# lauradarcy/gym-craftingworld

Measured on AMD Instinct MI355X. Metric: env-steps/sec at 65536 envs, 1/2/4/8 MI355X; bit-exact vs CPU ref, higher is better.
Workload: dtype u8

## Files before the change

gym_craftingworld_amd/_lib.py:

```python
import ctypes as C
import os

_HERE = os.path.dirname(os.path.abspath(__file__))
LIB_PATH = os.path.join(_HERE, 'libcraftingworld.so')


def lib_path():
    return os.environ.get('CW_LIB_PATH') or LIB_PATH

CW_ABI_VERSION = 5
CW_MT_N = 624
CW_MAX_TASKS = 16
CW_MAX_MENUS = 256

CW_OK, CW_ERR_INVALID, CW_ERR_HIP, CW_ERR_STATE = 0, -1, -2, -3
CW_OBS_STATE, CW_OBS_PIXELS_FULL, CW_OBS_PIXELS_DIRTY = 0, 1, 2
CW_ACT_I32, CW_ACT_I64, CW_ACT_U8 = 0, 1, 2
CW_RASTER_RAY, CW_RASTER_ALT = 0, 1


class cw_task_menu(C.Structure):
    _fields_ = [('n_selected', C.c_int32), ('number_of_tasks', C.c_int32), ('stacking', C.c_int32),
                ('reward_subset', C.c_int32), ('selected_bits', C.c_int32 * CW_MAX_TASKS)]

# ... 46 lines not shown
    'cw_imagine_masked': (C.c_int, [_VP, _VP, _VP, C.c_int32, _VP, _VP, _VP]),
    'cw_sample_state_masked': (C.c_int, [_VP, _VP, C.c_int32, _VP, _VP]),
    'cw_step': (C.c_int, [_VP, _VP, C.c_int, _VP]),
    'cw_step_many': (C.c_int, [_VP, _VP, C.c_int, C.c_int32, _VP]),
    'cw_rollout': (C.c_int, [_VP, _VP, C.c_int32, _VP, _VP, _VP]),
    'cw_render': (C.c_int, [_VP, _VP, _VP]),
    'cw_render_onehot': (C.c_int, [_VP, _VP, C.c_int32, _VP, _VP]),
    'cw_export_grid': (C.c_int, [_VP, _VP, _VP]),
    'cw_export_onehot': (C.c_int, [_VP, _VP, _VP]),
    'cw_export_onehot_of': (C.c_int, [_VP, C.c_int, _VP, _VP]),
    'cw_get_state': (C.c_int, [_VP, C.POINTER(cw_state_view)]),
    'cw_set_state': (C.c_int, [_VP, C.POINTER(cw_state_view)]),
    'cw_checkpoint_bytes': (C.c_size_t, [_VP]),
    'cw_checkpoint_save': (C.c_int, [_VP, _VP, C.c_size_t]),
    'cw_checkpoint_load': (C.c_int, [_VP, _VP, C.c_size_t]),
    'cw_profile_begin': (C.c_int, [_VP, C.c_int]),
    'cw_profile_end': (C.c_int, [_VP, C.POINTER(cw_profile)]),
    'cw_tuner': (C.c_int, [_VP, C.POINTER(cw_tuner_state)]),
    'cw_step_resident': (C.c_int, [_VP, C.c_int32, C.c_int32]),
    'cw_resident_stop': (C.c_int, [_VP]),
    'cw_render_kernel_name': (C.c_char_p, [_VP]),
    'cw_buffers': (C.c_int, [_VP, C.POINTER(cw_buffer_table)]),
    'cw_synchronize': (C.c_int, [_VP, _VP]),
    'cw_num_envs': (C.c_int, [_VP]),
    'cw_abi_version': (C.c_int, []),
    'cw_last_error': (C.c_char_p, []),
}
class cwh_guard(C.Structure):
    _fields_ = [('rate', C.c_double), ('rate_top', C.c_double), ('ms_sum', C.c_double), ('prev_mean', C.c_double), ('ref_ms', C.c_double),
                ('ref_prev', C.c_double), ('ms_n', C.c_int32), ('late', C.c_int32), ('good', C.c_int32), ('slowdowns', C.c_int32),
                ('probes', C.c_int32), ('probe_need', C.c_int32), ('recover_need', C.c_int32), ('probing', C.c_int32), ('recovering', C.c_int32)]


class cwh_tuning(C.Structure):
    _fields_ = [(f, C.c_int32) for f in ('render_chunk_rounds', 'step_envs_per_wave', 'gather', 'gather_max_size', 'small_frame_bytes',
                                         'small_blocks_per_cu', 'small_launch_mb', 'reset_blocks_per_cu', 'guard', 'verbose', 'lookahead',
                                         'la_period', 'rollout_segment', 'pad')] + \
              [(f, C.c_double) for f in ('head_notch', 'busy_notch', 'period_ns', 'rate_tbs')]


cwh_lookup = C.CFUNCTYPE(_VP, _VP, C.c_char_p)

CWH_GUARD_NONE, CWH_GUARD_SLOWDOWN, CWH_GUARD_TRIAL_UP, CWH_GUARD_TRIAL_KEPT, CWH_GUARD_TRIAL_UNDONE = range(5)
CWH_CKPT_SECTIONS = 22

HOST_HELPERS = {
    'cwh_mt_from_numpy': (C.c_int, [_VP, C.c_int]),
    'cwh_mt_to_numpy': (None, [_VP, C.c_int, _VP]),
    'cwh_mt_init_genrand': (None, [_VP, C.c_uint32]),
    'cwh_mt_untwist': (None, [_VP]),
    'cwh_mt_rewind': (None, [_VP, C.POINTER(C.c_int32), C.c_uint32]),
    'cwh_dlpack_make': (_VP, [_VP, C.c_int, C.c_int, C.c_int, C.c_int, C.POINTER(C.c_int64)]),
    'cwh_slots_to_grid': (None, [_VP, C.c_uint32, C.c_int, _VP]),
    'cwh_ckpt_section_bytes': (C.c_int, [C.c_int64, C.c_int32, C.c_int32, C.POINTER(C.c_size_t), C.POINTER(C.c_uint64)]),
    'cwh_guard_init': (None, [C.POINTER(cwh_guard), C.c_double]),
    'cwh_guard_step': (C.c_int, [C.POINTER(cwh_guard), C.c_double, C.c_double]),
    'cwh_sweep_periods': (None, [C.c_double, C.c_int32, C.c_double, C.c_double, C.POINTER(C.c_int32), C.POINTER(C.c_int32), C.POINTER(C.c_int32)]),
    'cwh_guard_scheduled_ms': (C.c_double, [C.c_double, C.c_int32, C.c_int32, C.c_double]),
    'cwh_la_adapt': (C.c_int32, [C.c_int32, C.c_int32, C.c_uint64, C.POINTER(C.c_int32)]),
    'cwh_read_tuning': (None, [cwh_lookup, _VP, C.POINTER(cwh_tuning)]),
}


def bind_host_helpers(lib):
    for name, (res, args) in HOST_HELPERS.items():
        fn = getattr(lib, name)
        fn.restype = res
        fn.argtypes = args
    return lib

_libs = {}
_lib = None


class CraftingWorldError(RuntimeError):
    pass


def load():
    global _lib
    path = lib_path()
    if path in _libs:
        _lib = _libs[path]
        return _lib
    if not os.path.exists(path):
        raise CraftingWorldError(
            'HIP extension %s is missing; build it (python -c "import __graft_entry__ as g; g.build()"). '
            'There is no CPU fallback.' % path)
    try:
        import torch
    except ImportError:
# ... 21 lines not shown
```

gym_craftingworld_amd/csrc/cw_engine.cpp:

```cpp
#include <hip/hip_runtime.h>

#include <cstdarg>
#include <climits>
#include <cstdio>
#include <cstdlib>
#include <cstring>
#include <new>
#include <algorithm>
#include <vector>

#include "../../include/craftingworld.h"
#include "cw_layout.h"
#include "cw_host.h"

extern "C" {
hipError_t cwk_launch_step(const CwParams *P, const CwTuning *T, const void *actions, int act_dtype, int obs_mode, int auto_reset, hipStream_t st,
                           hipEvent_t *ev);
hipError_t cwk_launch_refill(const CwParams *P, const CwTuning *T, int all_envs, hipStream_t st);
hipError_t cwk_launch_reset_all(const CwParams *P, const CwTuning *T, int obs_mode, hipStream_t st);
hipError_t cwk_launch_reset_masked(const CwParams *P, const CwTuning *T, const uint8_t *mask, int obs_mode, hipStream_t st);
hipError_t cwk_launch_imagine_masked(const CwParams *P, const CwTuning *T, const uint8_t *mask, const uint16_t *desired, int commit, int obs_mode,
                                     uint8_t *out_frames, uint8_t *out_onehot, hipStream_t st);
hipError_t cwk_launch_sample_state_masked(const CwParams *P, const CwTuning *T, const uint8_t *mask, int pooled, uint16_t *out_cells, hipStream_t st);
hipError_t cwk_launch_pool(const CwParams *P, const CwTuning *T, hipStream_t st);
hipError_t cwk_launch_seed(const CwParams *P, const uint32_t *seeds_dev, hipStream_t st);
hipError_t cwk_launch_resident(const CwParams *P, CwResident *R, uint32_t seq0, int paint_dirty, unsigned long long idle_ticks,
                               unsigned long long life_ticks, hipStream_t st);
hipError_t cwk_launch_render_onehot(const CwParams *P, const uint8_t *onehot, int n_states, uint16_t *out, hipStream_t st);
hipError_t cwk_launch_render_restore(const CwParams *P, const CwTuning *T, hipStream_t st);
hipError_t cwk_launch_rollout(const CwParams *P, const uint8_t *actions, int T, int32_t *rewards, uint8_t *dones, hipStream_t st);
hipError_t cwk_launch_render_ext(const CwParams *P, const CwTuning *T, uint8_t *out, hipStream_t st);
hipError_t cwk_launch_sweep_calib(const CwParams *P, const CwTuning *T, hipStream_t st);
void cwk_sweep_shape(const CwParams *P, const CwTuning *T, int *n_chunks, int *waves, int *jobs_per_wave);
hipError_t cwk_launch_idle(hipStream_t st);
hipError_t cwk_launch_export(const CwParams *P, const CwTuning *T, uint8_t *out, int onehot, int which, hipStream_t st);
}

#include <time.h>

static thread_local char g_err[512] = "";

static int fail(int code, const char *fmt, ...)
{
    va_list ap;
    va_start(ap, fmt);
    vsnprintf(g_err, sizeof(g_err), fmt, ap);
    va_end(ap);
    return code;
}

// ... 125 lines not shown
{
    void *p = nullptr;
    size_t bytes = count * sizeof(T);
    if (bytes == 0) bytes = 16;
    HIP_TRY(hipMalloc(&p, bytes));
    HIP_TRY(hipMemset(p, 0, bytes));
    e->allocs.push_back(p);
    *out = (T *)p;
    return CW_OK;
}

template <typename T>
static int host_alloc(cw_engine *e, T **out, size_t count)
{
    void *p = nullptr, *d = nullptr;
    size_t bytes = count * sizeof(T);
    if (bytes == 0) bytes = 16;
    HIP_TRY(hipHostMalloc(&p, bytes, hipHostMallocCoherent));
    e->host_allocs.push_back(p);
    memset(p, 0, bytes);
    HIP_TRY(hipHostGetDevicePointer(&d, p, 0));
    if (d != p) return fail(CW_ERR_HIP, "cw_create: mapped host memory has a different device address (no unified addressing)");
    *out = (T *)p;
    return CW_OK;
}

static void prof_free(cw_engine *e)
{
    for (hipEvent_t ev : e->prof_ev) (void)hipEventDestroy(ev);
    e->prof_ev.clear();
    e->prof_cap = e->prof_n = 0;
}

static int timed_render_stats(cw_engine *e, double *median, double *p90, double *mean = nullptr)
{
    enum { LAUNCHES = 24, SKIP = 4 };
    hipEvent_t evs[2 * LAUNCHES] = {};
    bool ok = true;
    for (hipEvent_t &ev : evs) ok = ok && hipEventCreate(&ev) == hipSuccess;
    for (int rep = 0; rep < LAUNCHES && ok; rep++)
        ok = hipEventRecord(evs[2 * rep], e->aux) == hipSuccess && cwk_launch_sweep_calib(&e->P, &e->tune, e->aux) == hipSuccess &&
             hipEventRecord(evs[2 * rep + 1], e->aux) == hipSuccess && cwk_launch_idle(e->aux) == hipSuccess;
    ok = ok && hipStreamSynchronize(e->aux) == hipSuccess;
    float ms[LAUNCHES];
    for (int rep = 0; rep < LAUNCHES && ok; rep++) ok = hipEventElapsedTime(&ms[rep], evs[2 * rep], evs[2 * rep + 1]) == hipSuccess;
    for (hipEvent_t &ev : evs) if (ev) (void)hipEventDestroy(ev);
    if (!ok) return fail(CW_ERR_HIP, "cw_create: render calibration failed");
    std::sort(ms + SKIP, ms + LAUNCHES);
    const int n = LAUNCHES - SKIP;
    *median = ms[SKIP + n / 2];
    *p90 = ms[SKIP + (9 * n) / 10 - 1];
    if (mean) { double acc = 0; for (int i = SKIP; i < LAUNCHES; i++) acc += ms[i]; *mean = acc / n; }
    return CW_OK;
}

static double sweep_period_ns(const cw_engine *e, double tb_per_s) { return (double)e->sweep_waves * 4096.0 / (tb_per_s * 1e12) * 1e9; }
static void set_sweep_rate(cw_engine *e, double tb_per_s)
{
    cwh_sweep_periods(tb_per_s, e->sweep_waves, e->head_notch, e->busy_notch, &e->tune.period16, &e->tune.period16_head, &e->tune.period16_busy);
}

static int calibrate_sweep(cw_engine *e)
{
    CwTuning &tn = e->tune;
    int n_chunks = 1, jobs_per_wave = 1;
    cwk_sweep_shape(&e->P, &tn, &n_chunks, &e->sweep_waves, &jobs_per_wave);
    e->sweep_jobs = (double)n_chunks * jobs_per_wave;
    if (e->tune_period_ns >= 0) {
        const double ns = e->tune_period_ns;
        set_sweep_rate(e, ns > 0 ? (double)e->sweep_waves * 4096.0 / (ns * 1e-9) * 1e-12 : 0.0);
        if (ns > 0) tn.period16 = (int)(ns * 1.6 + 0.5);
        return CW_OK;
    }
    set_sweep_rate(e, 7.0);
    if (e->host_actions) { set_sweep_rate(e, 0); return CW_OK; }
    if (e->obs_mode != CW_OBS_PIXELS_FULL || (double)e->n * e->P.frame_bytes < (double)(64ll << 20)) return CW_OK;
    static const double rates[] = {7.7, 7.4, 7.2, 7.0, 6.8, 6.6, 0.0};
    char log[1024] = "";
    size_t len = 0;
    int rc = CW_OK;
    double best_p90 = 0, med = 0, p90 = 0, mean = 0;
    rc = timed_render_stats(e, &med, &p90);
    set_sweep_rate(e, 6.4);
    if (rc == CW_OK) rc = timed_render_stats(e, &med, &p90);
    e->sweep_beside_ms = med - e->sweep_jobs * sweep_period_ns(e, 6.4) * 1e-6;
    if (e->tune_rate_tbs >= 0) e->sweep_rate = e->tune_rate_tbs;
    for (size_t i = 0; i < sizeof(rates) / sizeof(rates[0]) && rc == CW_OK && e->tune_rate_tbs < 0; i++) {
        set_sweep_rate(e, rates[i]);
        rc = timed_render_stats(e, &med, &p90, &mean);
        if (len < sizeof(log) - 56) len += (size_t)snprintf(log + len, sizeof(log) - len, " %.1f TB/s (%.0f ns): %.4f/%.4f/%.4f |", rates[i], tn.period16 / 1.6, med, p90, mean);
        if (rc == CW_OK && (best_p90 == 0 || p90 < 0.995 * best_p90)) { best_p90 = p90; e->sweep_rate = rates[i]; }
    }
    set_sweep_rate(e, e->sweep_rate);
    cwh_guard_init(&e->guard, e->sweep_rate);
    e->guard_on = rc == CW_OK && e->sweep_rate > 0 && e->auto_reset && e->tune_guard;
    if (e->guard_on)
        for (auto &smp : e->guard_ring)
            for (hipEvent_t &ev : smp.ev)
                if (hipEventCreate(&ev) != hipSuccess) e->guard_on = false;
    if (e->verbose)
        fprintf(stderr, "[craftingworld] sweep clock, ms per sweep (median/90th percentile/mean of 20; 0.0 TB/s = unclocked):%s -> %s%.0f ns\n", log,
                tn.period16 ? "" : "unclocked, ", tn.period16 / 1.6);
    return rc;
}

enum { CW_GUARD_EVERY = 64 };
static hipEvent_t *sweep_guard_tick(cw_engine *e, hipStream_t st)
{
    if (++e->guard_step % CW_GUARD_EVERY) return nullptr;
    while (e->guard_tail != e->guard_head && hipEventQuery(e->guard_ring[e->guard_tail % cw_engine::GUARD_RING].ev[5]) == hipSuccess) {
        cw_engine::GuardSample &smp = e->guard_ring[e->guard_tail++ % cw_engine::GUARD_RING];
        float ms = 0.f;
        if (hipEventElapsedTime(&ms, smp.ev[4], smp.ev[5]) != hipSuccess || ms <= 0.f || smp.period16 != e->tune.period16) continue;
        const double scheduled = cwh_guard_scheduled_ms(e->sweep_jobs, e->tune.period16, e->tune.period16_busy, e->sweep_beside_ms);
        const double rate_before = e->guard.rate, prev_mean = e->guard.prev_mean;
        const int recovering = e->guard.recovering;
        const int action = cwh_guard_step(&e->guard, ms, scheduled);
        if (e->guard.rate != rate_before) set_sweep_rate(e, e->guard.rate);
        if (e->verbose && action != CWH_GUARD_NONE) {
            static const char *what[] = {"", "three samples in a row late: a notch down", "trying a notch up", "the trial pays: kept", "the trial does not pay: undone"};
            fprintf(stderr, "[craftingworld] sweep clock: %s%s -- %.4f ms against %.4f scheduled (mean at the rate left %.4f): %.1f -> %.1f TB/s (%.0f ns)\n", what[action],
                    recovering ? " (on the way back to the best rate known)" : "", ms, scheduled, prev_mean, rate_before, e->guard.rate, e->tune.period16 / 1.6);
        }
    }
    if (e->guard_head - e->guard_tail >= (unsigned)cw_engine::GUARD_RING) return nullptr;
    cw_engine::GuardSample &slot = e->guard_ring[e->guard_head++ % cw_engine::GUARD_RING];
    slot.period16 = e->tune.period16;
    return slot.ev;
}

static void read_tuning(cw_engine *e)
{
    CwTuning &tn = e->tune;
    cwh_tuning t{};
    t.render_chunk_rounds = tn.render_chunk_rounds;
// ... 394 lines not shown
    if (!e->has_reset) return fail(CW_ERR_STATE, "cw_sample_state_masked called before cw_reset");
    DeviceGuard guard(e->device);
    if (!guard.ok) return fail(CW_ERR_HIP, "hipSetDevice(%d) failed", e->device);
    PARK(e);
    const int rc = rewind_streams(e, (hipStream_t)stream, "cw_sample_state_masked");
    if (rc != CW_OK) return rc;
    if (stream_capturing((hipStream_t)stream)) e->captured = true; else note_work(e, (hipStream_t)stream);
    HIP_TRY(cwk_launch_sample_state_masked(&e->P, &e->tune, mask, pooled != 0, out_cells, (hipStream_t)stream));
    if (e->res && hipEventRecord(e->last_work, (hipStream_t)stream) == hipSuccess) e->last_work_set = true;
    return CW_OK;
}

int cw_step(cw_engine *e, const void *actions, int action_dtype, cw_stream_t stream)
{
    if (!e || !actions) return fail(CW_ERR_INVALID, "cw_step: null argument");
    if (action_dtype < CW_ACT_I32 || action_dtype > CW_ACT_U8) return fail(CW_ERR_INVALID, "cw_step: bad action dtype %d", action_dtype);
    if (!e->has_reset) return fail(CW_ERR_STATE, "cw_step called before cw_reset");
    DeviceGuard guard(e->device);
    if (!guard.ok) return fail(CW_ERR_HIP, "hipSetDevice(%d) failed", e->device);
    PARK(e);
    const bool capturing = e->in_step_many ? e->capturing_now : stream_capturing((hipStream_t)stream);
    if (capturing) e->captured = true;
    else if (e->n_work != 1 || e->work[0] != (hipStream_t)stream) note_work(e, (hipStream_t)stream);
    hipEvent_t *ev = (e->prof_n < e->prof_cap) ? &e->prof_ev[(size_t)e->prof_n * 6] : nullptr;
    const bool profiled = ev != nullptr;
    if (e->guard_on && !ev && !capturing) ev = sweep_guard_tick(e, (hipStream_t)stream);
    if (capturing && e->P.lookahead && !e->la_refill_all && e->la_steps + 1 < e->la_period && !e->in_step_many) e->la_steps = e->la_period;
    if (e->P.lookahead && (e->la_refill_all || ++e->la_steps >= e->la_period)) {
        if (e->la_feedback && !capturing) la_adapt(e);
        HIP_TRY(cwk_launch_refill(&e->P, &e->tune, e->la_refill_all ? 1 : 0, (hipStream_t)stream));
        e->la_refill_all = false;
        e->la_steps = 0;
    }
    HIP_TRY(cwk_launch_step(&e->P, &e->tune, actions, action_dtype, e->obs_mode, e->auto_reset, (hipStream_t)stream, ev));
    if (profiled) e->prof_n++;
    if (e->res && hipEventRecord(e->last_work, (hipStream_t)stream) == hipSuccess) e->last_work_set = true;
    return CW_OK;
}

int cw_step_many(cw_engine *e, const void *actions, int action_dtype, int32_t n_steps, cw_stream_t stream)
{
    if (!e || !actions) return fail(CW_ERR_INVALID, "cw_step_many: null argument");
    if (n_steps < 1) return fail(CW_ERR_INVALID, "cw_step_many: n_steps must be >= 1");
    if (action_dtype < CW_ACT_I32 || action_dtype > CW_ACT_U8) return fail(CW_ERR_INVALID, "cw_step_many: bad action dtype %d", action_dtype);
    e->capturing_now = stream_capturing((hipStream_t)stream);
    if (e->P.lookahead && e->capturing_now) e->la_steps = e->la_period;
    const size_t row = (size_t)e->n * (action_dtype == CW_ACT_I32 ? 4 : action_dtype == CW_ACT_I64 ? 8 : 1);
    e->in_step_many = true;
    int rc = CW_OK;
    for (int32_t t = 0; t < n_steps && rc == CW_OK; t++) rc = cw_step(e, (const unsigned char *)actions + (size_t)t * row, action_dtype, stream);
    e->in_step_many = false;
    return rc;
}

int cw_step_resident(cw_engine *e, int32_t action, int32_t want_onehot)
{
    if (!e) return fail(CW_ERR_INVALID, "cw_step_resident: null engine");
    if (!e->res) return fail(CW_ERR_INVALID, "cw_step_resident needs num_envs == 1, host_outputs, auto_reset == 0 and obs_mode state or pixels_dirty");
    if (!e->has_reset) return fail(CW_ERR_STATE, "cw_step_resident called before cw_reset");
    if (action < 0 || action > 127) return fail(CW_ERR_INVALID, "cw_step_resident: action %d outside 0..127", action);
    if (want_onehot && !e->P.res_onehot) return fail(CW_ERR_INVALID, "cw_step_resident: no host one-hot buffer on this engine");
    CwResident *R = e->res;
    const uint32_t seq = (++e->res_seq) & 0xFFFFFFu;
    __atomic_store_n(&R->bell, (unsigned long long)((seq << 8) | (want_onehot ? 0x80u : 0u) | (uint32_t)action), __ATOMIC_RELEASE);
    struct timespec t0;
    clock_gettime(CLOCK_MONOTONIC, &t0);
    for (unsigned spins = 0;; spins++) {
// ... 556 lines not shown
```

gym_craftingworld_amd/csrc/cw_host.cpp:

```cpp
#include "cw_host.h"

#include <algorithm>
#include <cerrno>
#include <climits>
#include <cmath>
#include <cstdlib>
#include <cstring>

static inline uint32_t mt_twist(uint32_t cur, uint32_t nxt, uint32_t far)
{
    const uint32_t y = (cur & 0x80000000u) | (nxt & 0x7fffffffu);
    return far ^ (y >> 1) ^ ((y & 1u) ? 0x9908b0dfu : 0u);
}

extern "C" {

int cwh_mt_from_numpy(uint32_t *s, int pos)
{
    if (pos < 0) pos = 0;
    if (pos > CWH_MT_N) pos = CWH_MT_N;
    for (int k = 0; k < pos; k++)
        s[k] = mt_twist(s[k], s[(k + 1) % CWH_MT_N], s[(k + 397) % CWH_MT_N]);
    return pos % CWH_MT_N;
}
// ... 148 lines not shown
    if (g->probing && (g->late >= 3 || (verdict_due && mean >= 0.998 * g->prev_mean))) {
        const double ref_prev = g->ref_prev;
        guard_set_rate(g, g->rate - CWH_GUARD_NOTCH);
        g->ref_ms = ref_prev;
        int32_t &need = g->recovering ? g->recover_need : g->probe_need;
        need = std::min(2 * need, (int32_t)CWH_GUARD_NEED_MAX);
        g->probing = g->recovering = 0;
        return CWH_GUARD_TRIAL_UNDONE;
    }
    if (verdict_due) {
        if (g->recovering) g->recover_need = CWH_GUARD_RECOVER;
        else { g->rate_top = g->rate; g->probe_need = CWH_GUARD_RECOVER / 4; }
        g->ref_ms = mean;
        g->probing = g->recovering = 0;
        return CWH_GUARD_TRIAL_KEPT;
    }
    if (!g->probing && g->late >= 3 && g->rate > CWH_GUARD_RATE_FLOOR + 0.1) {
        guard_set_rate(g, g->rate - CWH_GUARD_NOTCH);
        g->slowdowns++;
        return CWH_GUARD_SLOWDOWN;
    }
    if (!g->probing && g->ms_n >= CWH_GUARD_PROBE_SAMPLES && g->rate + 0.05 < CWH_GUARD_RATE_CEILING &&
        g->good >= (g->rate + 0.1 < g->rate_top ? g->recover_need : g->probe_need)) {
        g->recovering = g->rate + 0.1 < g->rate_top;
        g->prev_mean = mean;
        g->ref_prev = g->ref_ms;
        guard_set_rate(g, std::min(g->rate + CWH_GUARD_NOTCH, CWH_GUARD_RATE_CEILING));
        g->probing = 1;
        if (!g->recovering) g->probes++;
        return CWH_GUARD_TRIAL_UP;
    }
    return CWH_GUARD_NONE;
}

int32_t cwh_la_adapt(int32_t period, int32_t period_max, uint64_t slow_delta, int32_t *quiet)
{
    if (slow_delta * 8ull > (uint64_t)period) {
        *quiet = 0;
        if (period > CWH_LA_PERIOD_MIN) period = period / 2 < CWH_LA_PERIOD_MIN ? CWH_LA_PERIOD_MIN : period / 2;
    } else if (slow_delta * 32ull <= (uint64_t)period && ++*quiet >= CWH_LA_QUIET) {
        *quiet = 0;
        if (period < period_max) period = period * 2 > period_max ? period_max : period * 2;
    }
    return period;
}

}

static bool tail_is_blank(const char *end)
{
    while (*end == ' ' || (*end >= '\t' && *end <= '\r')) end++;
    return *end == '\0';
}
static void tune_int(cwh_lookup lookup, void *ctx, const char *name, int32_t *field, long lo, long hi)
{
    const char *s = lookup(ctx, name);
    if (!s) return;
    char *end = nullptr;
    errno = 0;
    const long v = strtol(s, &end, 10);
    if (end == s || errno == ERANGE || !tail_is_blank(end) || v < lo || v > hi) return;
    *field = (int32_t)v;
}
static void tune_real(cwh_lookup lookup, void *ctx, const char *name, double *field, double lo)
{
    const char *s = lookup(ctx, name);
// ... 33 lines not shown
```

gym_craftingworld_amd/csrc/cw_host.h:

```cpp
#pragma once
#include <stddef.h>
#include <stdint.h>

#define CWH_MT_N 624

#ifdef __cplusplus
extern "C" {
#endif

int cwh_mt_from_numpy(uint32_t *s, int pos);
void cwh_mt_to_numpy(const uint32_t *s, int idx, uint32_t *key);
void cwh_mt_untwist(uint32_t *key);
void cwh_mt_rewind(uint32_t *key, int32_t *pos, uint32_t n);
void cwh_mt_init_genrand(uint32_t *s, uint32_t seed);

void *cwh_dlpack_make(void *data, int device_id, int code, int bits, int ndim, const int64_t *shape);

void cwh_slots_to_grid(const uint16_t *pos, uint32_t codes, int ncell, uint8_t *grid);

#define CWH_CKPT_SECTIONS 22
int cwh_ckpt_section_bytes(int64_t n, int32_t k, int32_t la_depth, size_t *sizes, uint64_t *total);

typedef struct cwh_guard {
    double rate;
    double rate_top;
    double ms_sum;
    double prev_mean;
    double ref_ms;
    double ref_prev;
    int32_t ms_n;
    int32_t late;
    int32_t good;
    int32_t slowdowns;
    int32_t probes;
    int32_t probe_need;
    int32_t recover_need;
    int32_t probing;
    int32_t recovering;
} cwh_guard;

enum { CWH_GUARD_NONE = 0, CWH_GUARD_SLOWDOWN = 1, CWH_GUARD_TRIAL_UP = 2, CWH_GUARD_TRIAL_KEPT = 3, CWH_GUARD_TRIAL_UNDONE = 4 };
#define CWH_GUARD_RECOVER 64
#define CWH_GUARD_PROBE_SAMPLES 32
#define CWH_GUARD_NEED_MAX 2048
#define CWH_GUARD_RATE_FLOOR 5.0
#define CWH_GUARD_RATE_CEILING 7.7
#define CWH_GUARD_NOTCH 0.2

void cwh_guard_init(cwh_guard *g, double rate);
int cwh_guard_step(cwh_guard *g, double ms, double scheduled_ms);
#define CWH_HEAD_JOBS 64
void cwh_sweep_periods(double rate, int32_t sweep_waves, double head_notch, double busy_notch, int32_t *period16, int32_t *period16_head, int32_t *period16_busy);
double cwh_guard_scheduled_ms(double sweep_jobs, int32_t period16, int32_t period16_busy, double beside_ms);

#define CWH_LA_PERIOD_MIN 8
#define CWH_LA_QUIET 8
int32_t cwh_la_adapt(int32_t period, int32_t period_max, uint64_t slow_delta, int32_t *quiet);

typedef struct cwh_tuning {
    int32_t render_chunk_rounds;
    int32_t step_envs_per_wave;
    int32_t gather;
    int32_t gather_max_size;
    int32_t small_frame_bytes;
    int32_t small_blocks_per_cu;
    int32_t small_launch_mb;
    int32_t reset_blocks_per_cu;
    int32_t guard;
    int32_t verbose;
    int32_t lookahead;
    int32_t la_period;
    int32_t rollout_segment;
    int32_t pad;
    double head_notch;
    double busy_notch;
    double period_ns;
    double rate_tbs;
} cwh_tuning;
typedef const char *(*cwh_lookup)(void *ctx, const char *name);
void cwh_read_tuning(cwh_lookup lookup, void *ctx, cwh_tuning *t);

#ifdef __cplusplus
}
#endif
```

gym_craftingworld_amd/csrc/cw_kernels.hip:

```cpp
#include <hip/hip_runtime.h>
#include <stdint.h>

#include "cw_layout.h"
#include "cw_mt.h"

#define CW_WAVE 64
#define CW_BALLOT(p) __builtin_amdgcn_ballot_w64(p)
#define CW_ALT_FRAME_PACE 2

#ifdef CW_TRACE
__device__ unsigned long long cw_trace_buf[1024 * 8];
#define CW_STAMP(env, k) do { if (lane == 0) { cw_trace_buf[((env) & 1023) * 8 + (k)] = wall_clock64(); \
                                               if ((k) == 0 || (k) == 5) cw_trace_buf[((env) & 1023) * 8 + 6 + ((k) ? 1 : 0)] = clock64(); } } while (0)
extern "C" hipError_t cwk_trace_read(unsigned long long *dst) { return hipMemcpyFromSymbol(dst, HIP_SYMBOL(cw_trace_buf), sizeof(cw_trace_buf)); }
#else
#define CW_STAMP(env, k) do { } while (0)
#endif

enum { EMPTY = 0, STICKS = 1, AXE = 2, HAMMER = 3, ROCK = 4, TREE = 5, BREAD = 6, HOUSE = 7, WHEAT = 8 };
enum { T_MAKEBREAD = 0, T_EATBREAD = 1, T_BUILDHOUSE = 2, T_CHOPTREE = 3, T_CHOPROCK = 4,
       T_GOTOHOUSE = 5, T_MOVEAXE = 6, T_MOVEHAMMER = 7, T_MOVESTICKS = 8 };

typedef uint32_t u32x3 __attribute__((ext_vector_type(3)));
typedef u32x3 u32x3_a4 __attribute__((aligned(4)));
// ... 1751 lines not shown
        const int env_n = min(per, P.n_envs - c * per);
        const long long pieces = ((long long)env_n * P.frame_bytes + CW_PIECE - 1) / CW_PIECE;
        if (cw_use_gather(P, tn)) {
            const int grid = cw_sweep_blocks(P, tn, pieces);
            if (cw_frames_per_job(P.frame_bytes) <= 4)
                hipLaunchKernelGGL(cw_render_gather_kernel<4>, dim3(grid), dim3(256), 0, st, P, frames, src, tn.period16, c * per, env_n);
            else
                hipLaunchKernelGGL(cw_render_gather_kernel<8>, dim3(grid), dim3(256), 0, st, P, frames, src, tn.period16, c * per, env_n);
            continue;
        }
        hipLaunchKernelGGL(k, dim3(cw_sweep_blocks(P, tn, pieces)), dim3(256), 0, st, P, frames, src, tn.period16, tn.period16_head, tn.period16_busy, (c == 0 ? 1 : 0) | (c == n_chunks - 1 ? 2 : 0), c * per, env_n);
    }
}

static inline int cw_wave_blocks(int waves) { return (waves + CW_RESET_WAVES - 1) / CW_RESET_WAVES; }
static inline int cw_reset_grid(const CwTuning &tn, int jobs)
{
    int blocks = cw_wave_blocks(jobs);
    if (blocks > tn.n_cu * tn.reset_blocks_per_cu) blocks = tn.n_cu * tn.reset_blocks_per_cu;
    if (blocks < 1) blocks = 1;
    return blocks;
}

static int cw_envs_per_wave(int n, int most = 64)
{
    int epw = most;
    while (epw > 8 && (n + epw - 1) / epw < 1024) epw >>= 1;
    return epw;
}

extern "C" {

hipError_t cwk_launch_step(const CwParams *P, const CwTuning *T, const void *actions, int act_dtype, int obs_mode,
                           int auto_reset, hipStream_t st, hipEvent_t *ev )
{
    const CwTuning &tn = *T;
    const int n = P->n_envs;
    const bool ev_all = ev && obs_mode != 1;
    if (ev_all) (void)hipEventRecord(ev[0], st);
    if (auto_reset) {
        const int epw = cw_envs_per_wave(n, tn.step_envs_per_wave);
        const int waves = (n + epw - 1) / epw;
        const int paint = obs_mode == 2 ? 1 : obs_mode == 1 ? 2 : 0;
        hipLaunchKernelGGL(cw_step_fused_variant(paint, paint != 0 && P->terminal_img != nullptr), dim3(cw_wave_blocks(waves)), dim3(CW_RESET_WAVES * CW_WAVE),
                           0, st, *P, actions, act_dtype, epw);
    } else {
        hipLaunchKernelGGL(cw_step_kernel, dim3((n + 255) / 256), dim3(256), 0, st, *P, actions, act_dtype, obs_mode == 2 ? 1 : 0);
    }
    if (ev_all) (void)hipEventRecord(ev[1], st);
    if (ev) for (int k = 2; k < 5; k++) (void)hipEventRecord(ev[k], st);
    if (obs_mode == 1) cw_launch_sweep(*P, tn, P->obs, CW_SRC_CURRENT, st);
    if (ev) (void)hipEventRecord(ev[5], st);
    return hipGetLastError();
}

hipError_t cwk_launch_refill(const CwParams *P, const CwTuning *T, int all_envs, hipStream_t st)
{
    hipLaunchKernelGGL(cw_refill_kernel, dim3(cw_reset_grid(*T, P->n_envs)), dim3(CW_RESET_WAVES * CW_WAVE), 0, st, *P, all_envs);
    return hipGetLastError();
}

hipError_t cwk_launch_rollout(const CwParams *P, const uint8_t *actions, int T, int32_t *rewards, uint8_t *dones, hipStream_t st)
{
    const int epw = cw_envs_per_wave(P->n_envs);
    const int waves = (P->n_envs + epw - 1) / epw;
    hipLaunchKernelGGL(cw_rollout_kernel, dim3(cw_wave_blocks(waves)), dim3(CW_RESET_WAVES * CW_WAVE), 0, st, *P, actions, T, rewards, dones, epw);
    return hipGetLastError();
}

hipError_t cwk_launch_render_restore(const CwParams *P, const CwTuning *T, hipStream_t st)
{
    cw_launch_sweep(*P, *T, P->obs, CW_SRC_CURRENT, st);
    cw_launch_sweep(*P, *T, P->init_img, CW_SRC_INIT, st);
    cw_launch_sweep(*P, *T, P->desired_img, CW_SRC_GOAL, st);
    return hipGetLastError();
}

hipError_t cwk_launch_reset_all(const CwParams *P, const CwTuning *T, int obs_mode, hipStream_t st)
{
    hipLaunchKernelGGL(cw_reset_kernel, dim3(cw_reset_grid(*T, P->n_envs)), dim3(CW_RESET_WAVES * CW_WAVE), 0, st, *P);
    if (obs_mode != 0) return cwk_launch_render_restore(P, T, st);
    return hipGetLastError();
}
// ... 116 lines not shown
```

Before: 309.0 million.

## Refine sweep-rate calibration with sustained-row stage and trim guard event records

Replaces the one-pass coarse sweep-rate table calibration with a staged host state machine. It keeps the coarse table, then measures a yardstick at a fixed rate, then runs interleaved sustained rows of batched launches at finer rates above the coarse pick, rejecting rates whose sub-rows saturate the scheduled time. It also stops recording unused step and idle events on non-profiled steps when the guard is active, creating only the two sweep events it reads. The aim is a rate that holds under sustained load and fewer event records per step, at the cost of a longer create-time calibration.

After: 307.0 million. About the same (-0.6%).

```diff
diff --git a/gym_craftingworld_amd/_lib.py b/gym_craftingworld_amd/_lib.py
--- a/gym_craftingworld_amd/_lib.py
+++ b/gym_craftingworld_amd/_lib.py
@@ -102,6 +102,12 @@
                 ('probes', C.c_int32), ('probe_need', C.c_int32), ('recover_need', C.c_int32), ('probing', C.c_int32), ('recovering', C.c_int32)]
 
 
+class cwh_calib(C.Structure):
+    _fields_ = [(f, C.c_double) for f in ('jobs', 'head_notch', 'busy_notch', 'r1', 'best_p90', 'r1_med', 'pick', 'med', 'p90', 'mean', 'beside_row')] + \
+               [(f, C.c_double * 4) for f in ('rate2', 'sum2', 'worst2')] + [(f, C.c_int32 * 4) for f in ('subrows2', 'sat_rows2')] + \
+               [(f, C.c_int32) for f in ('waves', 'stage', 'idx', 'n2', 'launches', 'row_subrows')]
+
+
 class cwh_tuning(C.Structure):
     _fields_ = [(f, C.c_int32) for f in ('render_chunk_rounds', 'step_envs_per_wave', 'gather', 'gather_max_size', 'small_frame_bytes',
                                          'small_blocks_per_cu', 'small_launch_mb', 'reset_blocks_per_cu', 'guard', 'verbose', 'lookahead',
@@ -113,6 +119,8 @@
 
 CWH_GUARD_NONE, CWH_GUARD_SLOWDOWN, CWH_GUARD_TRIAL_UP, CWH_GUARD_TRIAL_KEPT, CWH_GUARD_TRIAL_UNDONE = range(5)
 CWH_CKPT_SECTIONS = 22
+CWH_CALIB_DONE, CWH_CALIB_COARSE, CWH_CALIB_YARDSTICK, CWH_CALIB_ROWS_STAGE = range(4)
+CWH_CALIB_MAX_LAUNCHES = 7 * 24 + 5 * 8 + 4 * 3 * 12 * 8
 
 HOST_HELPERS = {
     'cwh_mt_from_numpy': (C.c_int, [_VP, C.c_int]),
@@ -127,6 +135,10 @@
     'cwh_guard_step': (C.c_int, [C.POINTER(cwh_guard), C.c_double, C.c_double]),
     'cwh_sweep_periods': (None, [C.c_double, C.c_int32, C.c_double, C.c_double, C.POINTER(C.c_int32), C.POINTER(C.c_int32), C.POINTER(C.c_int32)]),
     'cwh_guard_scheduled_ms': (C.c_double, [C.c_double, C.c_int32, C.c_int32, C.c_double]),
+    'cwh_calib_init': (None, [C.POINTER(cwh_calib), C.c_int32, C.c_double, C.c_double, C.c_double, C.c_double]),
+    'cwh_calib_next': (C.c_int, [C.POINTER(cwh_calib), C.POINTER(C.c_double), C.POINTER(C.c_int32), C.POINTER(C.c_int32)]),
+    'cwh_calib_feed': (None, [C.POINTER(cwh_calib), C.POINTER(C.c_double), C.c_int32]),
+    'cwh_calib_pick': (C.c_double, [C.POINTER(cwh_calib)]),
     'cwh_la_adapt': (C.c_int32, [C.c_int32, C.c_int32, C.c_uint64, C.POINTER(C.c_int32)]),
     'cwh_read_tuning': (None, [cwh_lookup, _VP, C.POINTER(cwh_tuning)]),
 }
diff --git a/gym_craftingworld_amd/csrc/cw_engine.cpp b/gym_craftingworld_amd/csrc/cw_engine.cpp
--- a/gym_craftingworld_amd/csrc/cw_engine.cpp
+++ b/gym_craftingworld_amd/csrc/cw_engine.cpp
@@ -15,7 +15,7 @@
 
 extern "C" {
 hipError_t cwk_launch_step(const CwParams *P, const CwTuning *T, const void *actions, int act_dtype, int obs_mode, int auto_reset, hipStream_t st,
-                           hipEvent_t *ev);
+                           hipEvent_t *ev, int ev_sweep_only);
 hipError_t cwk_launch_refill(const CwParams *P, const CwTuning *T, int all_envs, hipStream_t st);
 hipError_t cwk_launch_reset_all(const CwParams *P, const CwTuning *T, int obs_mode, hipStream_t st);
 hipError_t cwk_launch_reset_masked(const CwParams *P, const CwTuning *T, const uint8_t *mask, int obs_mode, hipStream_t st);
@@ -207,25 +207,39 @@
     e->prof_cap = e->prof_n = 0;
 }
 
-static int timed_render_stats(cw_engine *e, double *median, double *p90, double *mean = nullptr)
-{
-    enum { LAUNCHES = 24, SKIP = 4 };
-    hipEvent_t evs[2 * LAUNCHES] = {};
+static int timed_render_times(cw_engine *e, int launches, int per_time, double *ms)
+{
+    const int n = launches / per_time;
+    std::vector<hipEvent_t> evs(per_time == 1 ? (size_t)2 * n : (size_t)n + 1, nullptr);
     bool ok = true;
     for (hipEvent_t &ev : evs) ok = ok && hipEventCreate(&ev) == hipSuccess;
-    for (int rep = 0; rep < LAUNCHES && ok; rep++)
-        ok = hipEventRecord(evs[2 * rep], e->aux) == hipSuccess && cwk_launch_sweep_calib(&e->P, &e->tune, e->aux) == hipSuccess &&
-             hipEventRecord(evs[2 * rep + 1], e->aux) == hipSuccess && cwk_launch_idle(e->aux) == hipSuccess;
+    for (int rep = 0; rep < n * per_time && ok; rep++) {
+        if (per_time == 1 || rep % per_time == 0) ok = hipEventRecord(evs[per_time == 1 ? 2 * rep : rep / per_time], e->aux) == hipSuccess;
+        ok = ok && cwk_launch_sweep_calib(&e->P, &e->tune, e->aux) == hipSuccess;
+        if (per_time == 1) ok = ok && hipEventRecord(evs[2 * rep + 1], e->aux) == hipSuccess;
+        ok = ok && cwk_launch_idle(e->aux) == hipSuccess;
+    }
+    if (per_time > 1) ok = ok && hipEventRecord(evs[n], e->aux) == hipSuccess;
     ok = ok && hipStreamSynchronize(e->aux) == hipSuccess;
-    float ms[LAUNCHES];
-    for (int rep = 0; rep < LAUNCHES && ok; rep++) ok = hipEventElapsedTime(&ms[rep], evs[2 * rep], evs[2 * rep + 1]) == hipSuccess;
+    for (int i = 0; i < n && ok; i++) {
+        float t = 0.f;
+        ok = hipEventElapsedTime(&t, evs[per_time == 1 ? 2 * i : i], evs[per_time == 1 ? 2 * i + 1 : i + 1]) == hipSuccess;
+        ms[i] = (double)t / per_time;
+    }
     for (hipEvent_t &ev : evs) if (ev) (void)hipEventDestroy(ev);
     if (!ok) return fail(CW_ERR_HIP, "cw_create: render calibration failed");
+    return CW_OK;
+}
+static int timed_render_stats(cw_engine *e, double *median, double *p90)
+{
+    enum { LAUNCHES = CWH_CALIB_TABLE_LAUNCHES, SKIP = CWH_CALIB_TABLE_SKIP };
+    double ms[LAUNCHES];
+    const int rc = timed_render_times(e, LAUNCHES, 1, ms);
+    if (rc != CW_OK) return rc;
     std::sort(ms + SKIP, ms + LAUNCHES);
     const int n = LAUNCHES - SKIP;
     *median = ms[SKIP + n / 2];
     *p90 = ms[SKIP + (9 * n) / 10 - 1];
-    if (mean) { double acc = 0; for (int i = SKIP; i < LAUNCHES; i++) acc += ms[i]; *mean = acc / n; }
     return CW_OK;
 }
 
@@ -250,32 +264,45 @@
     set_sweep_rate(e, 7.0);
     if (e->host_actions) { set_sweep_rate(e, 0); return CW_OK; }
     if (e->obs_mode != CW_OBS_PIXELS_FULL || (double)e->n * e->P.frame_bytes < (double)(64ll << 20)) return CW_OK;
-    static const double rates[] = {7.7, 7.4, 7.2, 7.0, 6.8, 6.6, 0.0};
-    char log[1024] = "";
+    char log[1024] = "", log2[512] = "";
     size_t len = 0;
     int rc = CW_OK;
-    double best_p90 = 0, med = 0, p90 = 0, mean = 0;
+    double med = 0, p90 = 0;
     rc = timed_render_stats(e, &med, &p90);
     set_sweep_rate(e, 6.4);
     if (rc == CW_OK) rc = timed_render_stats(e, &med, &p90);
     e->sweep_beside_ms = med - e->sweep_jobs * sweep_period_ns(e, 6.4) * 1e-6;
-    if (e->tune_rate_tbs >= 0) e->sweep_rate = e->tune_rate_tbs;
-    for (size_t i = 0; i < sizeof(rates) / sizeof(rates[0]) && rc == CW_OK && e->tune_rate_tbs < 0; i++) {
-        set_sweep_rate(e, rates[i]);
-        rc = timed_render_stats(e, &med, &p90, &mean);
-        if (len < sizeof(log) - 56) len += (size_t)snprintf(log + len, sizeof(log) - len, " %.1f TB/s (%.0f ns): %.4f/%.4f/%.4f |", rates[i], tn.period16 / 1.6, med, p90, mean);
-        if (rc == CW_OK && (best_p90 == 0 || p90 < 0.995 * best_p90)) { best_p90 = p90; e->sweep_rate = rates[i]; }
-    }
+    cwh_calib cal;
+    cwh_calib_init(&cal, e->sweep_waves, e->sweep_jobs, e->head_notch, e->busy_notch, e->tune_rate_tbs);
+    double rate = 0, ms[CWH_CALIB_FEED_MAX];
+    int32_t launches = 0, per_time = 1;
+    for (int stage; rc == CW_OK && (stage = cwh_calib_next(&cal, &rate, &launches, &per_time)) != CWH_CALIB_DONE;) {
+        if (launches / per_time > CWH_CALIB_FEED_MAX) return fail(CW_ERR_INVALID, "cw_create: render calibration asked for too much");
+        set_sweep_rate(e, rate);
+        rc = timed_render_times(e, launches, per_time, ms);
+        if (rc != CW_OK) break;
+        cwh_calib_feed(&cal, ms, launches / per_time);
+        if (stage == CWH_CALIB_COARSE && len < sizeof(log) - 56)
+            len += (size_t)snprintf(log + len, sizeof(log) - len, " %.1f TB/s (%.0f ns): %.4f/%.4f/%.4f |", rate, tn.period16 / 1.6, cal.med, cal.p90, cal.mean);
+    }
+    e->sweep_rate = cwh_calib_pick(&cal);
+    len = 0;
+    for (int i = 0; i < cal.n2 && cal.subrows2[i] > 0 && len < sizeof(log2) - 64; i++)
+        len += (size_t)snprintf(log2 + len, sizeof(log2) - len, " %.1f TB/s: %.4f/%.3f/%d |", cal.rate2[i], cal.sum2[i] / cal.subrows2[i], cal.worst2[i], cal.sat_rows2[i]);
     set_sweep_rate(e, e->sweep_rate);
     cwh_guard_init(&e->guard, e->sweep_rate);
     e->guard_on = rc == CW_OK && e->sweep_rate > 0 && e->auto_reset && e->tune_guard;
     if (e->guard_on)
         for (auto &smp : e->guard_ring)
-            for (hipEvent_t &ev : smp.ev)
-                if (hipEventCreate(&ev) != hipSuccess) e->guard_on = false;
-    if (e->verbose)
-        fprintf(stderr, "[craftingworld] sweep clock, ms per sweep (median/90th percentile/mean of 20; 0.0 TB/s = unclocked):%s -> %s%.0f ns\n", log,
-                tn.period16 ? "" : "unclocked, ", tn.period16 / 1.6);
+            for (int k = 4; k < 6; k++)
+                if (hipEventCreate(&smp.ev[k]) != hipSuccess) e->guard_on = false;
+    if (e->verbose) {
+        fprintf(stderr, "[craftingworld] sweep clock, ms per sweep (median/90th percentile/mean of 20; 0.0 TB/s = unclocked):%s -> %.1f TB/s\n", log, cal.r1);
+        if (log2[0])
+            fprintf(stderr, "[craftingworld] sweep clock, sustained rows (%d x %d launches per rate in sub-rows of %d, %.4f ms beside the jobs; mean ms per launch/worst sub-row "
+                            "over its schedule/saturated rows):%s\n", CWH_CALIB_ROWS, cal.row_subrows * CWH_CALIB_SUBROW, CWH_CALIB_SUBROW, cal.beside_row, log2);
+        fprintf(stderr, "[craftingworld] sweep clock -> %s%.1f TB/s, %.0f ns (%d calibration launches)\n", tn.period16 ? "" : "unclocked, ", e->sweep_rate, tn.period16 / 1.6, cal.launches);
+    }
     return rc;
 }
 
@@ -736,7 +763,7 @@
         e->la_refill_all = false;
         e->la_steps = 0;
     }
-    HIP_TRY(cwk_launch_step(&e->P, &e->tune, actions, action_dtype, e->obs_mode, e->auto_reset, (hipStream_t)stream, ev));
+    HIP_TRY(cwk_launch_step(&e->P, &e->tune, actions, action_dtype, e->obs_mode, e->auto_reset, (hipStream_t)stream, ev, profiled ? 0 : 1));
     if (profiled) e->prof_n++;
     if (e->res && hipEventRecord(e->last_work, (hipStream_t)stream) == hipSuccess) e->last_work_set = true;
     return CW_OK;
diff --git a/gym_craftingworld_amd/csrc/cw_host.cpp b/gym_craftingworld_amd/csrc/cw_host.cpp
--- a/gym_craftingworld_amd/csrc/cw_host.cpp
+++ b/gym_craftingworld_amd/csrc/cw_host.cpp
@@ -204,6 +204,112 @@
     }
     return CWH_GUARD_NONE;
 }
+
+static const double calib_table[CWH_CALIB_TABLE] = {7.7, 7.4, 7.2, 7.0, 6.8, 6.6, 0.0};
+static double calib_grid(double rate) { return std::floor(rate * 10.0 + 0.5) / 10.0; }
+static double calib_scheduled_ms(const cwh_calib *c, double rate)
+{
+    int32_t p = 0, ph = 0, pb = 0;
+    cwh_sweep_periods(rate, c->waves, c->head_notch, c->busy_notch, &p, &ph, &pb);
+    return cwh_guard_scheduled_ms(c->jobs, p, pb, c->beside_row);
+}
+static void calib_end(cwh_calib *c, double pick)
+{
+    c->pick = pick;
+    c->stage = CWH_CALIB_DONE;
+}
+void cwh_calib_init(cwh_calib *c, int32_t sweep_waves, double sweep_jobs, double head_notch, double busy_notch, double forced_rate)
+{
+    memset(c, 0, sizeof(*c));
+    c->waves = sweep_waves;
+    c->jobs = sweep_jobs;
+    c->head_notch = head_notch;
+    c->busy_notch = busy_notch;
+    c->stage = CWH_CALIB_COARSE;
+    if (forced_rate >= 0) calib_end(c, forced_rate);
+}
+int cwh_calib_next(cwh_calib *c, double *rate, int32_t *launches, int32_t *per_time)
+{
+    switch (c->stage) {
+    case CWH_CALIB_COARSE:
+        *rate = calib_table[c->idx];
+        *launches = CWH_CALIB_TABLE_LAUNCHES;
+        *per_time = 1;
+        break;
+    case CWH_CALIB_YARDSTICK:
+        *rate = CWH_CALIB_YARD_RATE;
+        *launches = CWH_CALIB_YARD_SUBROWS * CWH_CALIB_SUBROW;
+        *per_time = CWH_CALIB_SUBROW;
+        break;
+    case CWH_CALIB_ROWS_STAGE:
+        *rate = c->rate2[c->idx % c->n2];
+        *launches = c->row_subrows * CWH_CALIB_SUBROW;
+        *per_time = CWH_CALIB_SUBROW;
+        break;
+    default:
+        return CWH_CALIB_DONE;
+    }
+    c->launches += *launches;
+    return c->stage;
+}
+void cwh_calib_feed(cwh_calib *c, const double *ms, int32_t n)
+{
+    if (c->stage == CWH_CALIB_COARSE && n == CWH_CALIB_TABLE_LAUNCHES) {
+        double t[CWH_CALIB_TABLE_LAUNCHES];
+        std::copy(ms, ms + n, t);
+        std::sort(t + CWH_CALIB_TABLE_SKIP, t + n);
+        const int cnt = n - CWH_CALIB_TABLE_SKIP;
+        c->med = t[CWH_CALIB_TABLE_SKIP + cnt / 2];
+        c->p90 = t[CWH_CALIB_TABLE_SKIP + (9 * cnt) / 10 - 1];
+        c->mean = 0;
+        for (int i = CWH_CALIB_TABLE_SKIP; i < n; i++) c->mean += t[i] / cnt;
+        if (c->best_p90 == 0 || c->p90 < 0.995 * c->best_p90) { c->best_p90 = c->p90; c->r1 = calib_table[c->idx]; c->r1_med = c->med; }
+        if (++c->idx < CWH_CALIB_TABLE) return;
+        if (c->r1 <= 0) { calib_end(c, 0.0); return; }
+        const double lo = c->r1 + 0.05 > CWH_GUARD_RATE_CEILING ? CWH_GUARD_RATE_CEILING - 0.2 : c->r1;
+        for (c->n2 = 0; c->n2 < CWH_CALIB_FINE && lo + 0.1 * c->n2 < CWH_GUARD_RATE_CEILING + 0.05; c->n2++) {
+            c->rate2[c->n2] = calib_grid(lo + 0.1 * c->n2);
+            c->worst2[c->n2] = 0;
+        }
+        const double fit = CWH_CALIB_ROWS_MS / (c->n2 * CWH_CALIB_ROWS * CWH_CALIB_SUBROW * std::max(c->r1_med, 1e-6));
+        c->row_subrows = fit >= CWH_CALIB_ROW_SUBROWS ? CWH_CALIB_ROW_SUBROWS : fit <= 3 ? 3 : (int32_t)fit;
+        c->idx = 0;
+        c->stage = CWH_CALIB_YARDSTICK;
+        return;
+    }
+    if (c->stage == CWH_CALIB_YARDSTICK && n == CWH_CALIB_YARD_SUBROWS) {
+        double t[CWH_CALIB_YARD_SUBROWS];
+        std::copy(ms, ms + n, t);
+        std::sort(t + 1, t + n);
+        int32_t p = 0, ph = 0, pb = 0;
+        cwh_sweep_periods(CWH_CALIB_YARD_RATE, c->waves, c->head_notch, c->busy_notch, &p, &ph, &pb);
+        c->beside_row = t[1 + (n - 1) / 2] - c->jobs * (p / 1.6) * 1e-6;
+        c->stage = CWH_CALIB_ROWS_STAGE;
+        return;
+    }
+    if (c->stage == CWH_CALIB_ROWS_STAGE && n == c->row_subrows) {
+        const int k = c->idx % c->n2;
+        const double scheduled = calib_scheduled_ms(c, c->rate2[k]);
+        bool saturated = false;
+        for (int i = 1; i < n; i++) {
+            c->sum2[k] += ms[i];
+            c->subrows2[k]++;
+            c->worst2[k] = std::max(c->worst2[k], ms[i] / scheduled);
+            saturated = saturated || ms[i] > 1.06 * scheduled;
+        }
+        c->sat_rows2[k] += saturated;
+        if (++c->idx < CWH_CALIB_ROWS * c->n2) return;
+        double best = 0;
+        for (int i = 0; i < c->n2; i++)
+            if (!c->sat_rows2[i] && (best == 0 || c->sum2[i] / c->subrows2[i] < best)) best = c->sum2[i] / c->subrows2[i];
+        for (int i = 0; i < c->n2; i++)
+            if (!c->sat_rows2[i] && c->sum2[i] / c->subrows2[i] <= 1.002 * best) { calib_end(c, c->rate2[i]); return; }
+        calib_end(c, c->r1);
+        return;
+    }
+    calib_end(c, c->r1 > 0 ? c->r1 : 0.0);
+}
+double cwh_calib_pick(const cwh_calib *c) { return c->pick; }
 
 int32_t cwh_la_adapt(int32_t period, int32_t period_max, uint64_t slow_delta, int32_t *quiet)
 {
diff --git a/gym_craftingworld_amd/csrc/cw_host.h b/gym_craftingworld_amd/csrc/cw_host.h
--- a/gym_craftingworld_amd/csrc/cw_host.h
+++ b/gym_craftingworld_amd/csrc/cw_host.h
@@ -53,6 +53,43 @@
 void cwh_sweep_periods(double rate, int32_t sweep_waves, double head_notch, double busy_notch, int32_t *period16, int32_t *period16_head, int32_t *period16_busy);
 double cwh_guard_scheduled_ms(double sweep_jobs, int32_t period16, int32_t period16_busy, double beside_ms);
 
+#define CWH_CALIB_TABLE 7
+#define CWH_CALIB_TABLE_LAUNCHES 24
+#define CWH_CALIB_TABLE_SKIP 4
+#define CWH_CALIB_SUBROW 8
+#define CWH_CALIB_ROW_SUBROWS 12
+#define CWH_CALIB_ROWS 3
+#define CWH_CALIB_ROWS_MS 250.0
+#define CWH_CALIB_YARD_SUBROWS 5
+#define CWH_CALIB_YARD_RATE 6.4
+#define CWH_CALIB_FINE 4
+#define CWH_CALIB_FEED_MAX 24
+#define CWH_CALIB_MAX_LAUNCHES (CWH_CALIB_TABLE * CWH_CALIB_TABLE_LAUNCHES + CWH_CALIB_YARD_SUBROWS * CWH_CALIB_SUBROW + \
+                                CWH_CALIB_FINE * CWH_CALIB_ROWS * CWH_CALIB_ROW_SUBROWS * CWH_CALIB_SUBROW)
+enum { CWH_CALIB_DONE = 0, CWH_CALIB_COARSE = 1, CWH_CALIB_YARDSTICK = 2, CWH_CALIB_ROWS_STAGE = 3 };
+typedef struct cwh_calib {
+    double jobs, head_notch, busy_notch;
+    double r1, best_p90, r1_med;
+    double pick;
+    double med, p90, mean;
+    double beside_row;
+    double rate2[CWH_CALIB_FINE];
+    double sum2[CWH_CALIB_FINE];
+    double worst2[CWH_CALIB_FINE];
+    int32_t subrows2[CWH_CALIB_FINE];
+    int32_t sat_rows2[CWH_CALIB_FINE];
+    int32_t waves;
+    int32_t stage;
+    int32_t idx;
+    int32_t n2;
+    int32_t launches;
+    int32_t row_subrows;
+} cwh_calib;
+void cwh_calib_init(cwh_calib *c, int32_t sweep_waves, double sweep_jobs, double head_notch, double busy_notch, double forced_rate);
+int cwh_calib_next(cwh_calib *c, double *rate, int32_t *launches, int32_t *per_time);
+void cwh_calib_feed(cwh_calib *c, const double *ms, int32_t n);
+double cwh_calib_pick(const cwh_calib *c);
+
 #define CWH_LA_PERIOD_MIN 8
 #define CWH_LA_QUIET 8
 int32_t cwh_la_adapt(int32_t period, int32_t period_max, uint64_t slow_delta, int32_t *quiet);
diff --git a/gym_craftingworld_amd/csrc/cw_kernels.hip b/gym_craftingworld_amd/csrc/cw_kernels.hip
--- a/gym_craftingworld_amd/csrc/cw_kernels.hip
+++ b/gym_craftingworld_amd/csrc/cw_kernels.hip
@@ -1807,11 +1807,11 @@
 extern "C" {
 
 hipError_t cwk_launch_step(const CwParams *P, const CwTuning *T, const void *actions, int act_dtype, int obs_mode,
-                           int auto_reset, hipStream_t st, hipEvent_t *ev )
+                           int auto_reset, hipStream_t st, hipEvent_t *ev , int ev_sweep_only )
 {
     const CwTuning &tn = *T;
     const int n = P->n_envs;
-    const bool ev_all = ev && obs_mode != 1;
+    const bool ev_all = ev && !ev_sweep_only && obs_mode != 1;
     if (ev_all) (void)hipEventRecord(ev[0], st);
     if (auto_reset) {
         const int epw = cw_envs_per_wave(n, tn.step_envs_per_wave);
@@ -1823,7 +1823,7 @@
         hipLaunchKernelGGL(cw_step_kernel, dim3((n + 255) / 256), dim3(256), 0, st, *P, actions, act_dtype, obs_mode == 2 ? 1 : 0);
     }
     if (ev_all) (void)hipEventRecord(ev[1], st);
-    if (ev) for (int k = 2; k < 5; k++) (void)hipEventRecord(ev[k], st);
+    if (ev) for (int k = ev_sweep_only ? 4 : 2; k < 5; k++) (void)hipEventRecord(ev[k], st);
     if (obs_mode == 1) cw_launch_sweep(*P, tn, P->obs, CW_SRC_CURRENT, st);
     if (ev) (void)hipEventRecord(ev[5], st);
     return hipGetLastError();
```
